# SysSec-KAIST/LTESniffer

Hardware: AMD Instinct MI355X
Metric: subframes/s (20 MHz, 150 RNTIs) (higher is better)
Workload: dtype f32+int16

## Files before the change

__graft_entry__.py:

```python
import os
import subprocess
import sys

os.environ.setdefault("GPU_MAX_HW_QUEUES", "16")

ROOT = os.path.dirname(os.path.abspath(__file__))
for p in (ROOT, os.path.join(ROOT, "tests")):
    if p not in sys.path:
        sys.path.insert(0, p)


def build():
    import ltesniffer_amd as la
    la.build(verbose=False)
    la.lib()
    for s in la.EXPORTS:
        getattr(la.lib(), s)
    subprocess.check_call(["make", "-C", os.path.join(ROOT, "oracle")], stdout=subprocess.DEVNULL)
    subprocess.check_call(["make", "-C", os.path.join(ROOT, "tools", "txgen")], stdout=subprocess.DEVNULL)
    subprocess.check_call(["make", "-C", os.path.join(ROOT, "tools", "pool_driver")], stdout=subprocess.DEVNULL)
    subprocess.check_call(["make", "-C", os.path.join(ROOT, "tests", "native")], stdout=subprocess.DEVNULL)
    if os.path.exists("/opt/rocm/lib/llvm/bin/clang++"):
        subprocess.check_call(["make", "-C", os.path.join(ROOT, "tests", "native"), "_build/test_turbo_core"], stdout=subprocess.DEVNULL)
    if os.path.isdir("/root/reference/lib/src/util"):
        subprocess.check_call(["make", "-C", os.path.join(ROOT, "oracle"), "-f", "Makefile.ref"], stdout=subprocess.DEVNULL)


def smoke():
    import numpy as np
    import torch
    assert torch.cuda.is_available(), "smoke() needs cuda:0"
    import ltesniffer_amd as la
    from lsn_testlib import scenario
    from parity import compare_taps, gen_subframes, gpu_records, oracle_records, run_oracle
    sc = scenario("small", seed=7)
    tti0, iq, _ = gen_subframes(sc, 12)
    _, per_sf, orecs = run_oracle(sc, tti0, iq)
    phy = la.Phy(nof_rx_antennas=sc["nof_rx"], max_batch=12, device=0, pcapwriter=la.PcapWriter(None))
    assert phy.setCell(sc["nof_prb"], sc["nof_ports"], sc["cell_id"])
    d_iq = torch.from_numpy(iq.view(np.float32)).to("cuda:0")
    phy.process_device(d_iq.data_ptr(), 12, tti0, 0, torch.cuda.current_stream().cuda_stream)
    bad = compare_taps(phy, per_sf, sc, 0, 12)
    assert not bad, bad[:3]
    g, o = gpu_records(phy), oracle_records(orecs)
    assert len(o) > 0 and g == o, "MAC-LTE record stream differs from the oracle (%d vs %d)" % (len(g), len(o))
    phy.close()
    print("smoke ok: %d PDUs bit-identical to the oracle" % len(o))


if __name__ == "__main__":
    build()
    if len(sys.argv) > 1 and sys.argv[1] == "smoke":
        smoke()
```

ltesniffer_amd/csrc/kernels/lsn_turbo_core.h:

```cpp
#pragma once
#include <stdint.h>
#include <type_traits>
#include "lsn_rm.h"
#ifndef LSN_NEG_METRIC
#define LSN_NEG_METRIC (-12000)
#define LSN_EXT_CLIP 2047
#endif

typedef short lsn_s2 __attribute__((ext_vector_type(2)));
typedef lsn_s2 s2;

#ifdef LSN_TURBO_RANGE_CHECK
#include <cstdio>
#include <cstdlib>
static inline s2 pk_chk(int x, int y, const char* what)
{
  if (x < -32768 || x > 32767 || y < -32768 || y > 32767) { std::fprintf(stderr, "int16 range exceeded in %s: %d %d\n", what, x, y); std::abort(); }
  return s2{(short)x, (short)y};
}
static inline s2 pka(s2 a, s2 b) { return pk_chk((int)a.x + (int)b.x, (int)a.y + (int)b.y, "add"); }
static inline s2 pks(s2 a, s2 b) { return pk_chk((int)a.x - (int)b.x, (int)a.y - (int)b.y, "sub"); }
#else
LSN_HD s2 pka(s2 a, s2 b) { return a + b; }
LSN_HD s2 pks(s2 a, s2 b) { return a - b; }
#endif
LSN_HD s2 pkmax(s2 a, s2 b) { return __builtin_elementwise_max(a, b); }
#ifdef LSN_TURBO_RANGE_CHECK
static inline s2 pka_sat(s2 a, s2 b)
{
  const int x = (int)a.x + (int)b.x, y = (int)a.y + (int)b.y;
  if (x > 32767 || y > 32767) { std::fprintf(stderr, "int16 range exceeded on the positive side in alpha + beta: %d %d\n", x, y); std::abort(); }
  return s2{(short)(x < -32768 ? -32768 : x), (short)(y < -32768 ? -32768 : y)};
}
#elif defined(__HIP_DEVICE_COMPILE__)
LSN_HD s2 pka_sat(s2 a, s2 b) { return __builtin_elementwise_add_sat(a, b); }
#else
static inline s2 pka_sat(s2 a, s2 b)
{
  const int x = (int)a.x + (int)b.x, y = (int)a.y + (int)b.y;
  return s2{(short)(x < -32768 ? -32768 : (x > 32767 ? 32767 : x)), (short)(y < -32768 ? -32768 : (y > 32767 ? 32767 : y))};
}
#endif
LSN_HD uint32_t pk_u32(s2 v) { return __builtin_bit_cast(uint32_t, v); }
LSN_HD s2 pk_s2(uint32_t w) { return __builtin_bit_cast(s2, w); }
#ifdef __HIP_DEVICE_COMPILE__
template <int AL, int AH, int BL, int BH>
__device__ __forceinline__ s2 pka_sel(s2 a, s2 b)
{
  s2 d;
  asm("v_pk_add_u16 %0, %1, %2 op_sel:[%3,%4] op_sel_hi:[%5,%6]" : "=v"(d) : "v"(a), "v"(b), "n"(AL), "n"(BL), "n"(AH), "n"(BH));
  return d;
}
template <int AL, int AH, int BL, int BH>
__device__ __forceinline__ s2 pks_sel(s2 a, s2 b)
{
  s2 d;
  asm("v_pk_sub_i16 %0, %1, %2 op_sel:[%3,%4] op_sel_hi:[%5,%6]" : "=v"(d) : "v"(a), "v"(b), "n"(AL), "n"(BL), "n"(AH), "n"(BH));
  return d;
}
#else
template <int AL, int AH, int BL, int BH>
static inline s2 pka_sel(s2 a, s2 b) { return pka(s2{AL ? a.y : a.x, AH ? a.y : a.x}, s2{BL ? b.y : b.x, BH ? b.y : b.x}); }
template <int AL, int AH, int BL, int BH>
static inline s2 pks_sel(s2 a, s2 b) { return pks(s2{AL ? a.y : a.x, AH ? a.y : a.x}, s2{BL ? b.y : b.x, BH ? b.y : b.x}); }
#endif

LSN_HD int lsn_ext_scale(int x)
{
  const int t = 3 * x;
  const int r = (t + (int)((uint32_t)t >> 30)) >> 2;
  return r < -LSN_EXT_CLIP ? -LSN_EXT_CLIP : (r > LSN_EXT_CLIP ? LSN_EXT_CLIP : r);
}

template <bool NORM>
LSN_HD void lsn_step_fwd_pk(s2* a, s2 q)
{
  const s2 gg = pka_sel<0, 1, 1, 0>(q, q);
  const s2 p = pk_s2(pk_u32(gg) & 0xFFFF0000u);
  const s2 x0 = pka_sel<0, 0, 0, 1>(a[0], p), y0 = pka_sel<0, 0, 1, 0>(a[1], p);
  const s2 x1 = pka_sel<0, 0, 0, 1>(a[2], q), y1 = pka_sel<0, 0, 1, 0>(a[3], q);
  const s2 x2 = pka_sel<1, 1, 1, 0>(a[0], q), y2 = pka_sel<1, 1, 0, 1>(a[1], q);
  const s2 x3 = pka_sel<1, 1, 1, 0>(a[2], p), y3 = pka_sel<1, 1, 0, 1>(a[3], p);
  a[0] = pkmax(x0, y0); a[1] = pkmax(x1, y1); a[2] = pkmax(x2, y2); a[3] = pkmax(x3, y3);
  if (NORM) {
    const s2 n = a[0];
    a[0] = pks_sel<0, 1, 0, 0>(a[0], n); a[1] = pks_sel<0, 1, 0, 0>(a[1], n); a[2] = pks_sel<0, 1, 0, 0>(a[2], n); a[3] = pks_sel<0, 1, 0, 0>(a[3], n);
  }
}

template <bool NORM = true>
LSN_HD void lsn_step_bwd_pk(s2* b, const s2* A, s2 q, s2* M0o, s2* M1o)
{
  const s2 G0 = __builtin_shufflevector(b[0], b[2], 0, 2), G1 = __builtin_shufflevector(b[0], b[2], 1, 3);
  const s2 G2 = __builtin_shufflevector(b[1], b[3], 0, 2), G3 = __builtin_shufflevector(b[1], b[3], 1, 3);
  const s2 S = pk_s2(pk_u32(q) & 0xFFFF0000u);
  const s2 T = pka_sel<0, 0, 0, 1>(q, S);
  const s2 u00 = pka(G0, S), u01 = pka(G1, S), u02 = pka_sel<0, 1, 1, 0>(G3, S), u03 = pka_sel<0, 1, 1, 0>(G2, S);
  const s2 u10 = pka_sel<0, 1, 1, 0>(G1, T), u11 = pka_sel<0, 1, 1, 0>(G0, T), u12 = pka(G2, T), u13 = pka(G3, T);
  *M0o = pkmax(pkmax(pka_sat(A[0], u00), pka_sat(A[1], u01)), pkmax(pka_sat(A[2], u02), pka_sat(A[3], u03)));
  *M1o = pkmax(pkmax(pka_sat(A[0], u10), pka_sat(A[1], u11)), pkmax(pka_sat(A[2], u12), pka_sat(A[3], u13)));
  b[0] = pkmax(u00, u10); b[1] = pkmax(u01, u11); b[2] = pkmax(u02, u12); b[3] = pkmax(u03, u13);
  if (NORM) {
    const s2 n = b[0];
    b[0] = pks_sel<0, 1, 0, 0>(b[0], n); b[1] = pks_sel<0, 1, 0, 0>(b[1], n); b[2] = pks_sel<0, 1, 0, 0>(b[2], n); b[3] = pks_sel<0, 1, 0, 0>(b[3], n);
  }
}
LSN_HD int16_t lsn_ext_one(s2 M0, s2 M1, s2 q)
{
  const s2 m0 = pkmax(M0, M0.yx), m1 = pkmax(M1, M1.yx);
  const int L = (int)m1.x - (int)m0.x;
  const int hard = L < 0 ? 0 : (L > 1 ? 1 : L);
  return (int16_t)(lsn_ext_scale(L - (int)q.x) * 2 + hard);
}
LSN_HD s2 lsn_sat_sub(s2 a, s2 b)
{
#ifdef __HIP_DEVICE_COMPILE__
  return __builtin_elementwise_sub_sat(a, b);
#else
  const int x = (int)a.x - (int)b.x, y = (int)a.y - (int)b.y;
  return s2{(short)(x < -32768 ? -32768 : (x > 32767 ? 32767 : x)), (short)(y < -32768 ? -32768 : (y > 32767 ? 32767 : y))};
#endif
}
LSN_HD s2 lsn_ext_two(s2 M0a, s2 M1a, s2 qa, s2 M0b, s2 M1b, s2 qb)
{
#ifdef __HIP_DEVICE_COMPILE__
  s2 r0, r1, r2, r3, out;
  asm("v_max_i16_sdwa %0, %5, %5 dst_sel:WORD_0 dst_unused:UNUSED_PAD src0_sel:WORD_0 src1_sel:WORD_1\n\t"
      "v_max_i16_sdwa %1, %6, %6 dst_sel:WORD_0 dst_unused:UNUSED_PAD src0_sel:WORD_0 src1_sel:WORD_1\n\t"
      "v_max_i16_sdwa %0, %7, %7 dst_sel:WORD_1 dst_unused:UNUSED_PRESERVE src0_sel:WORD_0 src1_sel:WORD_1\n\t"
      "v_max_i16_sdwa %1, %8, %8 dst_sel:WORD_1 dst_unused:UNUSED_PRESERVE src0_sel:WORD_0 src1_sel:WORD_1\n\t"
      "v_perm_b32 %3, %10, %9, %11\n\t"
      "v_pk_sub_i16 %2, %1, %0 clamp\n\t"
      "v_pk_sub_i16 %3, %2, %3 clamp\n\t"
      "v_pk_max_i16 %3, %3, %12\n\t"
      "v_pk_min_i16 %3, %3, %13\n\t"
      "v_pk_lshrrev_b16 %0, 14, %3 op_sel_hi:[0,1]\n\t"
      "v_pk_mad_u16 %0, %3, 3, %0 op_sel_hi:[1,0,1]\n\t"
      "v_pk_max_i16 %1, %2, 0\n\t"
      "v_pk_min_i16 %1, %1, 1 op_sel_hi:[1,0]\n\t"
      "v_pk_ashrrev_i16 %0, 1, %0 op_sel_hi:[0,1]\n\t"
      "v_and_or_b32 %4, %0, %14, %1"
      : "=&v"(r0), "=&v"(r1), "=&v"(r2), "=&v"(r3), "=&v"(out)
      : "v"(M0a), "v"(M1a), "v"(M0b), "v"(M1b), "v"(qa), "v"(qb), "s"(0x05040100u), "s"(0xF556F556u), "s"(0x0AAA0AAAu), "s"(0xFFFEFFFEu));
  return out;
#else
  const s2 m0a = pkmax(M0a, M0a.yx), m1a = pkmax(M1a, M1a.yx), m0b = pkmax(M0b, M0b.yx), m1b = pkmax(M1b, M1b.yx);
  const s2 m0 = s2{m0a.x, m0b.x}, m1 = s2{m1a.x, m1b.x};
  const s2 L = lsn_sat_sub(m1, m0);
  s2 x = lsn_sat_sub(L, s2{qa.x, qb.x});
  const s2 lim = s2{2730, 2730};
  x = __builtin_elementwise_min(pkmax(x, -lim), lim);
  const s2 neg = x >> 15;
  const s2 r = (x * (short)3 + (neg & (short)3)) >> 2;
  const s2 hard = __builtin_elementwise_min(pkmax(L, s2{0, 0}), s2{1, 1});
  return r * (short)2 + hard;
#endif
}

LSN_HD void lsn_pack_c(const int* m, s2* c)
{
  for (int k = 0; k < 4; k++) c[k] = s2{(short)m[k], (short)m[k + 4]};
}

struct TurboLds {
  uint32_t* spp;
  int16_t* ext;
  uint8_t* ckpt;
  int bias = 0, cw = 0, ch = 0;
};
LSN_HD void lsn_ckpt_store(uint8_t* area, int nt, int slot, int lane, const s2* a, int cw = 0, int ch = 0)
{
  uint32_t* w = (uint32_t*)(area + (size_t)(slot * 14 * nt));
  const int lw = lane + cw;
  w[lw] = pk_u32(a[1]); w[nt + lw] = pk_u32(a[2]); w[2 * nt + lw] = pk_u32(a[3]);
  ((int16_t*)(w + 3 * nt))[lane + ch] = a[0].y;
}
LSN_HD void lsn_ckpt_load(const uint8_t* area, int nt, int slot, int lane, s2* a, int cw = 0, int ch = 0)
{
  const uint32_t* w = (const uint32_t*)(area + (size_t)(slot * 14 * nt));
  const int lw = lane + cw;
  a[1] = pk_s2(w[lw]); a[2] = pk_s2(w[nt + lw]); a[3] = pk_s2(w[2 * nt + lw]);
  a[0] = s2{0, ((const int16_t*)(w + 3 * nt))[lane + ch]};
}

#ifdef __HIP_DEVICE_COMPILE__
#define LSN_UMUL24(a, b) __umul24(a, b)
#define LSN_MUL24(a, b) __mul24(a, b)
#else
#define LSN_UMUL24(a, b) ((uint32_t)(a) * (uint32_t)(b))
#define LSN_MUL24(a, b) ((int)(a) * (int)(b))
#endif
LSN_HD int tr_idx(int x, int W, int P, uint32_t magicW)
{
  const int q = (int)(LSN_UMUL24((uint32_t)x, magicW) >> 20);
  return LSN_MUL24(x - LSN_MUL24(q, W), P) + q;
}
LSN_HD int fld0(uint32_t w) { return (int)(w << 22) >> 22; }
LSN_HD int fld1(uint32_t w) { return (int)(w << 12) >> 22; }
LSN_HD int fld2(uint32_t w) { return (int)(w << 2) >> 22; }

LSN_HD uint32_t lsn_perm(uint32_t hi, uint32_t lo, uint32_t sel)
{
#ifdef __HIP_DEVICE_COMPILE__
  return __builtin_amdgcn_perm(hi, lo, sel);
#else
  const uint64_t v = ((uint64_t)hi << 32) | lo;
  uint32_t d = 0;
  for (int k = 0; k < 4; k++) d |= (uint32_t)((v >> (8 * ((sel >> (8 * k)) & 7u))) & 0xFFu) << (8 * k);
  return d;
#endif
}
template <int PF>
LSN_HD int lsn_par_field(uint32_t w)
{
#ifdef __HIP_DEVICE_COMPILE__
  return __builtin_amdgcn_sbfe((int)w, PF, 10);
#else
  return (int)(w << (22 - PF)) >> 22;
#endif
}
template <int PF>
LSN_HD void lsn_operands2(uint32_t ws0, uint32_t ws1, uint32_t es0, uint32_t es1, uint32_t wp0, uint32_t wp1, uint32_t* g0, uint32_t* g1)
{
  const s2 sys = (pk_s2(lsn_perm(ws1, ws0, 0x05040100u)) << 6) >> 6;
  const s2 apr = pk_s2(lsn_perm(es1, es0, 0x05040100u)) >> 1;
  const uint32_t sum = pk_u32(pka(sys, apr));
  *g0 = lsn_perm((uint32_t)lsn_par_field<PF>(wp0), sum, 0x05040100u);
  *g1 = lsn_perm((uint32_t)lsn_par_field<PF>(wp1), sum, 0x05040302u);
}

#include "lsn_turbo_cyc.h"

#ifndef TB_S
#define TB_S 16
#endif
#define TB_CKPT_BYTES ((size_t)3584)
static_assert(TB_S == 16, "the check-point area is sized for sub-blocks of 16 steps");

LSN_HD void lsn_turbo_il_fill(uint32_t* dst, int K, int f1, int f2)
{
  const int P = lsn_turbo_nwin(K), W = K / P;
  for (int i = 0; i < ((W + 1) / 2) * P; i++) dst[i] = 0;
  for (int w = 0; w < P; w++)
    for (int t = 0; t < W; t++) {
      const long long x = (long long)w * W + t;
      const int pi = (int)(((long long)f1 * x + (long long)f2 * x % K * x) % K);
      dst[(t >> 1) * P + w] |= (uint32_t)((pi % W) * P + pi / W) << (16 * (t & 1));
    }
}

template <bool IL>
LSN_HD void lsn_map_pass_lane(const TurboLds& m, const uint32_t* il, int nt, int wl, int K, int P, int W,
                              const s2* nii_a, const s2* nii_b, const s2* beta_tail, s2* a_end, s2* b_out)
{
  const int lane = wl;
  int wlb = wl + m.bias;
#ifdef __HIP_DEVICE_COMPILE__
#define LSN_LOCAL_ADDR(x) asm volatile("" : "+v"(x))
#else
#define LSN_LOCAL_ADDR(x) (void)(x)
#endif
  const uint32_t bias2 = (uint32_t)m.bias * 0x10001u;
  const int nsb = (W + TB_S - 1) / TB_S;
  s2 a[4], b[4];
  auto a_start = [&]() {
    if (wl == 0) {
      a[0] = s2{0, (short)LSN_NEG_METRIC};
      a[1] = a[2] = a[3] = s2{(short)LSN_NEG_METRIC, (short)LSN_NEG_METRIC};
    } else {
      for (int k = 0; k < 4; k++) a[k] = nii_a[k];
    }
  };
  a_start();
  uint32_t nx[TB_S / 2];
  uint32_t cur[TB_S / 2];
  const int wlast = (W - 1) >> 1;
  auto il_load = [&](int sb) {
#pragma unroll
    for (int u = 0; u < TB_S / 2; u++) {
      int t2 = sb * (TB_S / 2) + u;
      t2 = t2 < wlast ? t2 : wlast;
      nx[u] = (il + (uint32_t)(t2 * P))[wl] + bias2;
    }
  };
  if (IL) il_load(0);
  uint32_t g[TB_S];
  auto build2 = [&](int tb, int u) {
    const int nat0 = (tb + u) * P + wlb, nat1 = nat0 + P;
    if (IL) {
      const int i0 = (int)(cur[u >> 1] & 0xFFFFu), i1 = (int)(cur[u >> 1] >> 16);
      lsn_operands2<20>(m.spp[i0], m.spp[i1], (uint16_t)m.ext[i0], (uint16_t)m.ext[i1], m.spp[nat0], m.spp[nat1], &g[u], &g[u + 1]);
    } else {
      const uint32_t w0 = m.spp[nat0], w1 = m.spp[nat1];
      lsn_operands2<10>(w0, w1, (uint16_t)m.ext[nat0], (uint16_t)m.ext[nat1], w0, w1, &g[u], &g[u + 1]);
    }
  };
  for (int sb = 0; sb + 1 < nsb; sb++) {
    LSN_LOCAL_ADDR(wlb);
    if (sb >= 1) lsn_ckpt_store(m.ckpt, nt, sb - 1, lane, a, m.cw, m.ch);
    const int tb = sb * TB_S;
    if (IL) {
#pragma unroll
      for (int u = 0; u < TB_S / 2; u++) cur[u] = nx[u];
      il_load(sb + 1);
    }
#pragma unroll
    for (int u = 0; u < TB_S; u += 2) build2(tb, u);
#pragma unroll
    for (int u = 0; u < TB_S; u += 2) {
      lsn_step_fwd_pk<false>(a, pk_s2(g[u]));
      lsn_step_fwd_pk<true>(a, pk_s2(g[u + 1]));
    }
  }
  if (wl == P - 1) {
    for (int k = 0; k < 4; k++) b[k] = beta_tail[k];
  } else {
    for (int k = 0; k < 4; k++) b[k] = nii_b[k];
  }
  s2 A[TB_S][4];
  auto ext_index = [&](int tb, int u) { return IL ? (int)((u & 1) ? cur[u >> 1] >> 16 : cur[u >> 1] & 0xFFFFu) : (tb + u) * P + wlb; };
  for (int sb = nsb - 1; sb >= 0; sb--) {
    LSN_LOCAL_ADDR(wlb);
    const int tb = sb * TB_S, n = (tb + TB_S < W) ? TB_S : W - tb;
    if (sb + 1 < nsb) {
      if (sb == 0) {
        a_start();
      } else {
        lsn_ckpt_load(m.ckpt, nt, sb - 1, lane, a, m.cw, m.ch);
      }
    }
    if (IL) {
#pragma unroll
      for (int u = 0; u < TB_S / 2; u++) cur[u] = nx[u];
      if (sb > 0) il_load(sb - 1);
    }
    auto subblock = [&](auto fullc) {
      constexpr bool FULL = decltype(fullc)::value;
#pragma unroll
      for (int u = TB_S - 2; u >= 0; u -= 2)
        if (FULL || u < n) build2(tb, u);
      if constexpr (FULL) {
        auto fwd1 = [&](auto uc) {
          constexpr int u = decltype(uc)::value;
          A[u][0] = a[0]; A[u][1] = a[1]; A[u][2] = a[2]; A[u][3] = a[3];
          lsn_cyc_fwd<u % 7>(a, pk_s2(g[u]));
          if (u & 1) {
            const s2 n0 = a[0];
            a[0] = pks_sel<0, 1, 0, 0>(a[0], n0); a[1] = pks_sel<0, 1, 0, 0>(a[1], n0); a[2] = pks_sel<0, 1, 0, 0>(a[2], n0); a[3] = pks_sel<0, 1, 0, 0>(a[3], n0);
          }
        };
#define LSN_IC(n) std::integral_constant<int, n>{}
        fwd1(LSN_IC(0)); fwd1(LSN_IC(1)); fwd1(LSN_IC(2)); fwd1(LSN_IC(3)); fwd1(LSN_IC(4)); fwd1(LSN_IC(5)); fwd1(LSN_IC(6)); fwd1(LSN_IC(7));
        fwd1(LSN_IC(8)); fwd1(LSN_IC(9)); fwd1(LSN_IC(10)); fwd1(LSN_IC(11)); fwd1(LSN_IC(12)); fwd1(LSN_IC(13)); fwd1(LSN_IC(14)); fwd1(LSN_IC(15));
        if (sb == nsb - 1) {
          lsn_cyc_to_c<TB_S % 7>(a);
          const s2 nn = a[0];
          for (int k = 0; k < 4; k++) a_end[k] = pks_sel<0, 1, 0, 0>(a[k], nn);
        }
        lsn_cyc_from_c<TB_S % 7>(b);
        auto bwd2 = [&](auto uc) {
          constexpr int u = decltype(uc)::value;
          s2 M0a, M1a, M0b, M1b;
          lsn_cyc_bwd<u % 7, false>(b, A[u], pk_s2(g[u]), &M0a, &M1a);
          lsn_cyc_bwd<(u - 1) % 7, true>(b, A[u - 1], pk_s2(g[u - 1]), &M0b, &M1b);
          const s2 e = lsn_ext_two(M0a, M1a, pk_s2(g[u]), M0b, M1b, pk_s2(g[u - 1]));
          m.ext[ext_index(tb, u)] = e.x;
          m.ext[ext_index(tb, u - 1)] = e.y;
        };
        bwd2(LSN_IC(15)); bwd2(LSN_IC(13)); bwd2(LSN_IC(11)); bwd2(LSN_IC(9)); bwd2(LSN_IC(7)); bwd2(LSN_IC(5)); bwd2(LSN_IC(3)); bwd2(LSN_IC(1));
#undef LSN_IC
      } else {
#pragma unroll
        for (int u = 0; u < TB_S; u++) {
          if (u < n) {
            A[u][0] = a[0]; A[u][1] = a[1]; A[u][2] = a[2]; A[u][3] = a[3];
            if (u & 1) lsn_step_fwd_pk<true>(a, pk_s2(g[u])); else lsn_step_fwd_pk<false>(a, pk_s2(g[u]));
          }
        }
        if (sb == nsb - 1) {
          const s2 nn = a[0];
          for (int k = 0; k < 4; k++) a_end[k] = pks_sel<0, 1, 0, 0>(a[k], nn);
        }
#pragma unroll
        for (int u = TB_S - 1; u >= 0; u--) {
          if (u < n) {
            s2 M0, M1;
            lsn_step_bwd_pk(b, A[u], pk_s2(g[u]), &M0, &M1);
            m.ext[ext_index(tb, u)] = lsn_ext_one(M0, M1, pk_s2(g[u]));
          }
        }
      }
    };
    if (n == TB_S) subblock(std::true_type{}); else subblock(std::false_type{});
  }
  for (int k = 0; k < 4; k++) b_out[k] = b[k];
}
```

Measured before the change: 273,700.

## Place partial turbo sub-block at window start so later sub-blocks are full

Reorganises the per-lane MAP window traversal so that any remainder (partial) sub-block and odd-length padding sit at the start of the window instead of the end. Every sub-block except the first can then take the fully unrolled cyclic fast path, and the interleaver table is shifted by one slot for odd window lengths. The final forward step of the last full block is skipped unless the end state is needed. This adds index arithmetic and a more complex first-block path, with some risk to correctness at the edges.

```diff
diff --git a/__graft_entry__.py b/__graft_entry__.py
--- a/__graft_entry__.py
+++ b/__graft_entry__.py
@@ -22,6 +22,7 @@
     subprocess.check_call(["make", "-C", os.path.join(ROOT, "tests", "native")], stdout=subprocess.DEVNULL)
     if os.path.exists("/opt/rocm/lib/llvm/bin/clang++"):
         subprocess.check_call(["make", "-C", os.path.join(ROOT, "tests", "native"), "_build/test_turbo_core"], stdout=subprocess.DEVNULL)
+        subprocess.check_call(["make", "-C", os.path.join(ROOT, "tests", "native"), "-f", "turbo_subblocks.mk"], stdout=subprocess.DEVNULL)
     if os.path.isdir("/root/reference/lib/src/util"):
         subprocess.check_call(["make", "-C", os.path.join(ROOT, "oracle"), "-f", "Makefile.ref"], stdout=subprocess.DEVNULL)
 
diff --git a/ltesniffer_amd/csrc/kernels/lsn_turbo_core.h b/ltesniffer_amd/csrc/kernels/lsn_turbo_core.h
--- a/ltesniffer_amd/csrc/kernels/lsn_turbo_core.h
+++ b/ltesniffer_amd/csrc/kernels/lsn_turbo_core.h
@@ -239,13 +239,13 @@
 
 LSN_HD void lsn_turbo_il_fill(uint32_t* dst, int K, int f1, int f2)
 {
-  const int P = lsn_turbo_nwin(K), W = K / P;
+  const int P = lsn_turbo_nwin(K), W = K / P, o = W & 1;
   for (int i = 0; i < ((W + 1) / 2) * P; i++) dst[i] = 0;
   for (int w = 0; w < P; w++)
     for (int t = 0; t < W; t++) {
       const long long x = (long long)w * W + t;
       const int pi = (int)(((long long)f1 * x + (long long)f2 * x % K * x) % K);
-      dst[(t >> 1) * P + w] |= (uint32_t)((pi % W) * P + pi / W) << (16 * (t & 1));
+      dst[((t + o) >> 1) * P + w] |= (uint32_t)((pi % W) * P + pi / W) << (16 * ((t + o) & 1));
     }
 }
 
@@ -261,7 +261,10 @@
 #define LSN_LOCAL_ADDR(x) (void)(x)
 #endif
   const uint32_t bias2 = (uint32_t)m.bias * 0x10001u;
-  const int nsb = (W + TB_S - 1) / TB_S;
+  const int o = W & 1, We = W + o;
+  const int nsb = (We + TB_S - 1) / TB_S;
+  const int n0 = We - TB_S * (nsb - 1);
+  const bool full0 = n0 == TB_S && !o;
   s2 a[4], b[4];
   auto a_start = [&]() {
     if (wl == 0) {
@@ -274,19 +277,20 @@
   a_start();
   uint32_t nx[TB_S / 2];
   uint32_t cur[TB_S / 2];
-  const int wlast = (W - 1) >> 1;
+  const int wlast = (We >> 1) - 1;
   auto il_load = [&](int sb) {
+    const int w0 = sb ? (n0 >> 1) + (sb - 1) * (TB_S / 2) : 0;
 #pragma unroll
     for (int u = 0; u < TB_S / 2; u++) {
-      int t2 = sb * (TB_S / 2) + u;
+      int t2 = w0 + u;
       t2 = t2 < wlast ? t2 : wlast;
       nx[u] = (il + (uint32_t)(t2 * P))[wl] + bias2;
     }
   };
   if (IL) il_load(0);
   uint32_t g[TB_S];
-  auto build2 = [&](int tb, int u) {
-    const int nat0 = (tb + u) * P + wlb, nat1 = nat0 + P;
+  auto build2 = [&](int tb, int u, bool spare) {
+    const int nat1 = (tb + u + 1) * P + wlb, nat0 = spare ? nat1 : nat1 - P;
     if (IL) {
       const int i0 = (int)(cur[u >> 1] & 0xFFFFu), i1 = (int)(cur[u >> 1] >> 16);
       lsn_operands2<20>(m.spp[i0], m.spp[i1], (uint16_t)m.ext[i0], (uint16_t)m.ext[i1], m.spp[nat0], m.spp[nat1], &g[u], &g[u + 1]);
@@ -298,18 +302,31 @@
   for (int sb = 0; sb + 1 < nsb; sb++) {
     LSN_LOCAL_ADDR(wlb);
     if (sb >= 1) lsn_ckpt_store(m.ckpt, nt, sb - 1, lane, a, m.cw, m.ch);
-    const int tb = sb * TB_S;
+    const int tb = sb ? n0 - o + (sb - 1) * TB_S : -o;
     if (IL) {
 #pragma unroll
       for (int u = 0; u < TB_S / 2; u++) cur[u] = nx[u];
       il_load(sb + 1);
     }
-#pragma unroll
-    for (int u = 0; u < TB_S; u += 2) build2(tb, u);
-#pragma unroll
-    for (int u = 0; u < TB_S; u += 2) {
-      lsn_step_fwd_pk<false>(a, pk_s2(g[u]));
-      lsn_step_fwd_pk<true>(a, pk_s2(g[u + 1]));
+    if (sb > 0 || full0) {
+#pragma unroll
+      for (int u = 0; u < TB_S; u += 2) build2(tb, u, false);
+#pragma unroll
+      for (int u = 0; u < TB_S; u += 2) {
+        lsn_step_fwd_pk<false>(a, pk_s2(g[u]));
+        lsn_step_fwd_pk<true>(a, pk_s2(g[u + 1]));
+      }
+    } else {
+#pragma unroll
+      for (int u = 0; u < TB_S; u += 2)
+        if (u < n0) build2(tb, u, u == 0 && o);
+#pragma unroll
+      for (int u = 0; u < TB_S; u += 2) {
+        if (u < n0) {
+          if (u > 0 || !o) lsn_step_fwd_pk<false>(a, pk_s2(g[u]));
+          lsn_step_fwd_pk<true>(a, pk_s2(g[u + 1]));
+        }
+      }
     }
   }
   if (wl == P - 1) {
@@ -321,7 +338,7 @@
   auto ext_index = [&](int tb, int u) { return IL ? (int)((u & 1) ? cur[u >> 1] >> 16 : cur[u >> 1] & 0xFFFFu) : (tb + u) * P + wlb; };
   for (int sb = nsb - 1; sb >= 0; sb--) {
     LSN_LOCAL_ADDR(wlb);
-    const int tb = sb * TB_S, n = (tb + TB_S < W) ? TB_S : W - tb;
+    const int tb = sb ? n0 - o + (sb - 1) * TB_S : -o;
     if (sb + 1 < nsb) {
       if (sb == 0) {
         a_start();
@@ -336,23 +353,24 @@
     }
     auto subblock = [&](auto fullc) {
       constexpr bool FULL = decltype(fullc)::value;
-#pragma unroll
-      for (int u = TB_S - 2; u >= 0; u -= 2)
-        if (FULL || u < n) build2(tb, u);
       if constexpr (FULL) {
+#pragma unroll
+        for (int u = TB_S - 2; u >= 0; u -= 2) build2(tb, u, false);
         auto fwd1 = [&](auto uc) {
           constexpr int u = decltype(uc)::value;
           A[u][0] = a[0]; A[u][1] = a[1]; A[u][2] = a[2]; A[u][3] = a[3];
           lsn_cyc_fwd<u % 7>(a, pk_s2(g[u]));
           if (u & 1) {
-            const s2 n0 = a[0];
-            a[0] = pks_sel<0, 1, 0, 0>(a[0], n0); a[1] = pks_sel<0, 1, 0, 0>(a[1], n0); a[2] = pks_sel<0, 1, 0, 0>(a[2], n0); a[3] = pks_sel<0, 1, 0, 0>(a[3], n0);
+            const s2 n0_ = a[0];
+            a[0] = pks_sel<0, 1, 0, 0>(a[0], n0_); a[1] = pks_sel<0, 1, 0, 0>(a[1], n0_); a[2] = pks_sel<0, 1, 0, 0>(a[2], n0_); a[3] = pks_sel<0, 1, 0, 0>(a[3], n0_);
           }
         };
 #define LSN_IC(n) std::integral_constant<int, n>{}
         fwd1(LSN_IC(0)); fwd1(LSN_IC(1)); fwd1(LSN_IC(2)); fwd1(LSN_IC(3)); fwd1(LSN_IC(4)); fwd1(LSN_IC(5)); fwd1(LSN_IC(6)); fwd1(LSN_IC(7));
-        fwd1(LSN_IC(8)); fwd1(LSN_IC(9)); fwd1(LSN_IC(10)); fwd1(LSN_IC(11)); fwd1(LSN_IC(12)); fwd1(LSN_IC(13)); fwd1(LSN_IC(14)); fwd1(LSN_IC(15));
+        fwd1(LSN_IC(8)); fwd1(LSN_IC(9)); fwd1(LSN_IC(10)); fwd1(LSN_IC(11)); fwd1(LSN_IC(12)); fwd1(LSN_IC(13)); fwd1(LSN_IC(14));
+        A[15][0] = a[0]; A[15][1] = a[1]; A[15][2] = a[2]; A[15][3] = a[3];
         if (sb == nsb - 1) {
+          lsn_cyc_fwd<15 % 7>(a, pk_s2(g[15]));
           lsn_cyc_to_c<TB_S % 7>(a);
           const s2 nn = a[0];
           for (int k = 0; k < 4; k++) a_end[k] = pks_sel<0, 1, 0, 0>(a[k], nn);
@@ -371,27 +389,32 @@
 #undef LSN_IC
       } else {
 #pragma unroll
-        for (int u = 0; u < TB_S; u++) {
-          if (u < n) {
+        for (int u = TB_S - 2; u >= 0; u -= 2)
+          if (u < n0) build2(tb, u, u == 0 && o);
+#pragma unroll
+        for (int u = 0; u < TB_S; u += 2) {
+          if (u < n0) {
             A[u][0] = a[0]; A[u][1] = a[1]; A[u][2] = a[2]; A[u][3] = a[3];
-            if (u & 1) lsn_step_fwd_pk<true>(a, pk_s2(g[u])); else lsn_step_fwd_pk<false>(a, pk_s2(g[u]));
+            if (u > 0 || !o) lsn_step_fwd_pk<false>(a, pk_s2(g[u]));
+            A[u + 1][0] = a[0]; A[u + 1][1] = a[1]; A[u + 1][2] = a[2]; A[u + 1][3] = a[3];
+            if (u + 2 < n0) lsn_step_fwd_pk<true>(a, pk_s2(g[u + 1]));
           }
         }
-        if (sb == nsb - 1) {
-          const s2 nn = a[0];
-          for (int k = 0; k < 4; k++) a_end[k] = pks_sel<0, 1, 0, 0>(a[k], nn);
-        }
-#pragma unroll
-        for (int u = TB_S - 1; u >= 0; u--) {
-          if (u < n) {
+#pragma unroll
+        for (int u = TB_S - 2; u >= 0; u -= 2) {
+          if (u < n0) {
             s2 M0, M1;
-            lsn_step_bwd_pk(b, A[u], pk_s2(g[u]), &M0, &M1);
-            m.ext[ext_index(tb, u)] = lsn_ext_one(M0, M1, pk_s2(g[u]));
+            lsn_step_bwd_pk(b, A[u + 1], pk_s2(g[u + 1]), &M0, &M1);
+            m.ext[ext_index(tb, u + 1)] = lsn_ext_one(M0, M1, pk_s2(g[u + 1]));
+            if (u > 0 || !o) {
+              lsn_step_bwd_pk(b, A[u], pk_s2(g[u]), &M0, &M1);
+              m.ext[ext_index(tb, u)] = lsn_ext_one(M0, M1, pk_s2(g[u]));
+            }
           }
         }
       }
     };
-    if (n == TB_S) subblock(std::true_type{}); else subblock(std::false_type{});
+    if (sb > 0 || full0) subblock(std::true_type{}); else subblock(std::false_type{});
   }
   for (int k = 0; k < 4; k++) b_out[k] = b[k];
 }
```

Result: no change. 275,200 (median of 6 runs) (+0.6%).

## Move partial turbo sub-block to window start so the tail sub-block is full

Applied to the files above, without the earlier changes.

Sub-block boundaries are realigned so that any remainder of W/TB_S is placed in the first sub-block instead of the last. The backward pass starts at the last sub-block, so it now usually runs the fully unrolled 16-step path instead of the slower predicated partial path. The interleaver table layout and its fill routine are changed to match the new boundaries. The forward pass gains a predicated path for a short first block. The a_end capture is removed from the partial branch, which is a correctness risk if the hidden full branch does not produce it, for example when there is only one sub-block.

```diff
diff --git a/ltesniffer_amd/csrc/kernels/lsn_turbo_core.h b/ltesniffer_amd/csrc/kernels/lsn_turbo_core.h
--- a/ltesniffer_amd/csrc/kernels/lsn_turbo_core.h
+++ b/ltesniffer_amd/csrc/kernels/lsn_turbo_core.h
@@ -237,6 +237,29 @@
 #define TB_CKPT_BYTES ((size_t)3584)
 static_assert(TB_S == 16, "the check-point area is sized for sub-blocks of 16 steps");
 
+struct LsnSubBlock {
+  int start;
+  int len;
+  int word;
+};
+LSN_HD int lsn_turbo_nsb(int W) { return (W + TB_S - 1) / TB_S; }
+LSN_HD LsnSubBlock lsn_turbo_sb(int W, int sb)
+{
+  const int d = -W & (TB_S - 1);
+  const int start = sb * TB_S - d, word = sb * (TB_S / 2) - (d >> 1);
+  return LsnSubBlock{start > 0 ? start : 0, sb ? TB_S : TB_S - d, word > 0 ? word : 0};
+}
+LSN_HD int lsn_turbo_fwd_steps(int W)
+{
+  int n = 0;
+  for (int sb = 0; sb + 1 < lsn_turbo_nsb(W); sb++) n += lsn_turbo_sb(W, sb).len;
+  return n;
+}
+#ifndef LSN_FWD_SWEEP_COUNT
+#define LSN_FWD_SWEEP_COUNT(n) (void)0
+#endif
+LSN_HD int lsn_turbo_sb_of(int W, int t) { return (t + (-W & (TB_S - 1))) / TB_S; }
+
 LSN_HD void lsn_turbo_il_fill(uint32_t* dst, int K, int f1, int f2)
 {
   const int P = lsn_turbo_nwin(K), W = K / P;
@@ -245,7 +268,9 @@
     for (int t = 0; t < W; t++) {
       const long long x = (long long)w * W + t;
       const int pi = (int)(((long long)f1 * x + (long long)f2 * x % K * x) % K);
-      dst[(t >> 1) * P + w] |= (uint32_t)((pi % W) * P + pi / W) << (16 * (t & 1));
+      const LsnSubBlock b = lsn_turbo_sb(W, lsn_turbo_sb_of(W, t));
+      const int u = t - b.start;
+      dst[(b.word + (u >> 1)) * P + w] |= (uint32_t)((pi % W) * P + pi / W) << (16 * (u & 1));
     }
 }
 
@@ -261,7 +286,7 @@
 #define LSN_LOCAL_ADDR(x) (void)(x)
 #endif
   const uint32_t bias2 = (uint32_t)m.bias * 0x10001u;
-  const int nsb = (W + TB_S - 1) / TB_S;
+  const int nsb = lsn_turbo_nsb(W);
   s2 a[4], b[4];
   auto a_start = [&]() {
     if (wl == 0) {
@@ -274,14 +299,11 @@
   a_start();
   uint32_t nx[TB_S / 2];
   uint32_t cur[TB_S / 2];
-  const int wlast = (W - 1) >> 1;
   auto il_load = [&](int sb) {
-#pragma unroll
-    for (int u = 0; u < TB_S / 2; u++) {
-      int t2 = sb * (TB_S / 2) + u;
-      t2 = t2 < wlast ? t2 : wlast;
-      nx[u] = (il + (uint32_t)(t2 * P))[wl] + bias2;
-    }
+    const int w0 = lsn_turbo_sb(W, sb).word;
+#pragma unroll
+    for (int u = 0; u < TB_S / 2; u++)
+      nx[u] = (il + (uint32_t)((w0 + u) * P))[wl] + bias2;
   };
   if (IL) il_load(0);
   uint32_t g[TB_S];
@@ -298,18 +320,37 @@
   for (int sb = 0; sb + 1 < nsb; sb++) {
     LSN_LOCAL_ADDR(wlb);
     if (sb >= 1) lsn_ckpt_store(m.ckpt, nt, sb - 1, lane, a, m.cw, m.ch);
-    const int tb = sb * TB_S;
+    const LsnSubBlock s = lsn_turbo_sb(W, sb);
+    const int tb = s.start, n = s.len;
     if (IL) {
 #pragma unroll
       for (int u = 0; u < TB_S / 2; u++) cur[u] = nx[u];
       il_load(sb + 1);
     }
-#pragma unroll
-    for (int u = 0; u < TB_S; u += 2) build2(tb, u);
-#pragma unroll
-    for (int u = 0; u < TB_S; u += 2) {
-      lsn_step_fwd_pk<false>(a, pk_s2(g[u]));
-      lsn_step_fwd_pk<true>(a, pk_s2(g[u + 1]));
+    if (n == TB_S) {
+#pragma unroll
+      for (int u = 0; u < TB_S; u += 2) build2(tb, u);
+#pragma unroll
+      for (int u = 0; u < TB_S; u += 2) {
+        lsn_step_fwd_pk<false>(a, pk_s2(g[u]));
+        lsn_step_fwd_pk<true>(a, pk_s2(g[u + 1]));
+        LSN_FWD_SWEEP_COUNT(2);
+      }
+    } else {
+#pragma unroll
+      for (int u = 0; u < TB_S; u += 2)
+        if (u < n) build2(tb, u);
+#pragma unroll
+      for (int u = 0; u < TB_S; u += 2) {
+        if (u + 1 < n) {
+          lsn_step_fwd_pk<false>(a, pk_s2(g[u]));
+          lsn_step_fwd_pk<true>(a, pk_s2(g[u + 1]));
+          LSN_FWD_SWEEP_COUNT(2);
+        } else if (u < n) {
+          lsn_step_fwd_pk<true>(a, pk_s2(g[u]));
+          LSN_FWD_SWEEP_COUNT(1);
+        }
+      }
     }
   }
   if (wl == P - 1) {
@@ -321,7 +362,8 @@
   auto ext_index = [&](int tb, int u) { return IL ? (int)((u & 1) ? cur[u >> 1] >> 16 : cur[u >> 1] & 0xFFFFu) : (tb + u) * P + wlb; };
   for (int sb = nsb - 1; sb >= 0; sb--) {
     LSN_LOCAL_ADDR(wlb);
-    const int tb = sb * TB_S, n = (tb + TB_S < W) ? TB_S : W - tb;
+    const LsnSubBlock s = lsn_turbo_sb(W, sb);
+    const int tb = s.start, n = s.len;
     if (sb + 1 < nsb) {
       if (sb == 0) {
         a_start();
@@ -377,10 +419,6 @@
             if (u & 1) lsn_step_fwd_pk<true>(a, pk_s2(g[u])); else lsn_step_fwd_pk<false>(a, pk_s2(g[u]));
           }
         }
-        if (sb == nsb - 1) {
-          const s2 nn = a[0];
-          for (int k = 0; k < 4; k++) a_end[k] = pks_sel<0, 1, 0, 0>(a[k], nn);
-        }
 #pragma unroll
         for (int u = TB_S - 1; u >= 0; u--) {
           if (u < n) {
```

Result: faster. 269,600 before, 275,300 after (median of 6 runs) (+2.1%).
